# bioinfologics/w2rap-contigger

Hardware: AMD Instinct MI355X
Metric: step2_k60_canonical_kmers_per_s (higher is better)
Workload: dtype u64

## Files before the change

include/w2rap_step2.h:

```cpp
#ifndef W2RAP_STEP2_H_
#define W2RAP_STEP2_H_

#include <stddef.h>
#include <stdint.h>

#ifdef __cplusplus
extern "C" {
#endif

#define W2RAP_STEP2_ABI_VERSION 3

enum {
    W2RAP_OK = 0,
    W2RAP_E_ARG = 1,
    W2RAP_E_NO_DEVICE = 2,
    W2RAP_E_HIP = 3,
    W2RAP_E_STATE = 4,
    W2RAP_E_LIMIT = 5,
    W2RAP_E_GRAPH = 6,
    W2RAP_E_HINT = 7,
    W2RAP_E_IO = 8
};

enum { W2RAP_MEM_HOST = 0, W2RAP_MEM_DEVICE = 1 };
// ... 81 lines not shown
const char* w2rap_step2_last_error(const w2rap_step2_ctx*);
int w2rap_step2_set_reads(w2rap_step2_ctx*, const w2rap_reads* reads);
int w2rap_step2_count_kmers(w2rap_step2_ctx*, uint32_t min_qual, uint32_t min_freq, w2rap_step2_out* stats);
int w2rap_step2_count_kmers_passes(w2rap_step2_ctx*, uint32_t min_qual, uint32_t min_freq, uint32_t n_passes, w2rap_step2_out* stats);
int w2rap_step2_build_graph(w2rap_step2_ctx*, const w2rap_edge_hint* hint);
int w2rap_step2_path_reads(w2rap_step2_ctx*);
int w2rap_step2_fetch(w2rap_step2_ctx*, w2rap_step2_out* out);
void* w2rap_step2_stream(w2rap_step2_ctx*);

int w2rap_step2_trim(w2rap_step2_ctx*);

int w2rap_step2_copy_bench(w2rap_step2_ctx*, uint64_t nbytes, uint32_t reps, double* gb_per_s);
int w2rap_step2_device_copy(w2rap_step2_ctx*, void* dst, const void* src, uint64_t nbytes);
int w2rap_step2_copy_bench_form(void);

int    w2rap_step2_set_profiling(w2rap_step2_ctx*, int on);
size_t w2rap_step2_profile(w2rap_step2_ctx*, char* buf, size_t len, int reset);

int w2rap_step2_counts(w2rap_step2_ctx*, uint64_t out[8]);

int w2rap_step2_get_good_len(w2rap_step2_ctx*, uint16_t* out );
int w2rap_step2_get_table(w2rap_step2_ctx*, uint64_t* hi, uint64_t* lo, uint8_t* count, uint8_t* ctx,
                          int32_t* edge, uint32_t* off );

int      w2rap_step2_quality_windows(w2rap_step2_ctx*, uint32_t min_qual, uint64_t* n_kmers );
uint32_t w2rap_step2_default_buckets(uint64_t total_kmers, uint32_t multiple_of);
uint32_t w2rap_step2_record_bytes(void);
int w2rap_step2_partition(w2rap_step2_ctx*, uint32_t n_buckets, uint32_t n_parts, uint64_t* recs_per_part,
                          uint64_t* kmers_per_part);
int w2rap_step2_partition_range(w2rap_step2_ctx*, uint32_t n_buckets, uint32_t first_bucket, uint32_t end_bucket, uint32_t n_parts,
                                uint64_t* recs_per_part, uint64_t* kmers_per_part);
int w2rap_step2_count_pass(w2rap_step2_ctx*, uint32_t pass, uint32_t n_passes);
int w2rap_step2_partition_buffers(w2rap_step2_ctx*, void** d_records, void** d_bucket_counts, uint64_t* n_records);
int w2rap_step2_count_records(w2rap_step2_ctx*, uint32_t min_freq, uint32_t n_local_buckets, uint32_t n_segments,
                              const void* d_records, const void* d_counts, uint64_t total_kmers, w2rap_step2_out* stats);
int w2rap_step2_count_records_begin(w2rap_step2_ctx*, uint32_t min_freq, uint32_t n_local_buckets, uint32_t n_segments,
                                    const void* d_records, const void* d_counts, uint64_t total_kmers, uint32_t n_slices,
                                    int deferred);
int w2rap_step2_count_records_slices(w2rap_step2_ctx*);
int w2rap_step2_count_records_bounds(w2rap_step2_ctx*, uint32_t k, uint32_t* first_bucket, uint32_t* end_bucket);
int w2rap_step2_count_records_launch(w2rap_step2_ctx*, uint32_t k);
int w2rap_step2_count_records_slice(w2rap_step2_ctx*, uint32_t k, uint64_t* n_solid, uint64_t* n_chunks);
int w2rap_step2_count_records_end(w2rap_step2_ctx*, w2rap_step2_out* stats);
int w2rap_step2_solid_buffers(w2rap_step2_ctx*, void** d_hi, void** d_lo, void** d_cc, uint64_t* n);
int w2rap_step2_set_solid(w2rap_step2_ctx*, const void* d_hi, const void* d_lo, const void* d_cc, uint64_t n,
                          uint64_t M, uint64_t D, const uint64_t* hist101);
// ... 37 lines not shown
```

w2rap_contigger_amd/csrc/ctx.h:

```cpp
#pragma once
#include <hip/hip_runtime.h>
#include <stdint.h>
#include <stdio.h>
#include <stdlib.h>
#include <cstdlib>
#include <string>
#include <utility>
#include <vector>
#include "../../include/w2rap_step2.h"
#include "common.h"

namespace w2 {

struct Ctx;
}
struct w2rap_step2_ctx;
namespace w2 {
struct Ctx {
    int device = 0;
    hipStream_t stream = nullptr;
    hipStream_t stream2 = nullptr;
    unsigned long long* h_pinned = nullptr;
    std::string err;
    int sm_count = 256;
// ... 22 lines not shown
    uint64_t* d_shi = nullptr;
    uint64_t* d_slo = nullptr;
    uint32_t* d_scc = nullptr;
    Slot* d_table = nullptr;
    uint64_t tcap = 0;
    unsigned long long* d_filter32 = nullptr;
    uint64_t f32words = 0;
    uint8_t* d_sctx = nullptr;
    void* d_nbr = nullptr;
    bool wide_ids = false;
    uint64_t* d_chunk_start = nullptr;
    uint32_t* d_chunk_cnt = nullptr;
    uint64_t nchunks = 0;
    KRec* d_srec = nullptr;
    bool use_index = false;
    uint4* d_index = nullptr;
    uint64_t index_cap = 0, index_entries = 0;
    uint4* d_xindex = nullptr; uint64_t xindex_cap = 0, xindex_kmers = 0;
    bool index_prebuilt = false, bits_ready = false, filter_prebuilt = false;
    unsigned cs_ns = 0;
    unsigned cs_planned = 0;
    uint32_t cs_nbl = 0, cs_nseg = 0; const uint32_t* cs_recs = nullptr;
    bool cs_short_first = false;
    hipEvent_t cs_ev[16] = {};
    unsigned long long* cs_cnt = nullptr;
    uint64_t* cs_off = nullptr;
    uint32_t cs_chunk_cap = 0;
    uint8_t* d_unres = nullptr;
    bool fused_prune = false;
    std::vector<std::pair<uint64_t, uint64_t>> unfused_chunks;
    uint32_t* cs_defer = nullptr;
    uint64_t* g_hi = nullptr; uint64_t* g_lo = nullptr; uint32_t* g_cc = nullptr;
    uint64_t* g_cstart = nullptr; uint32_t* g_ccnt = nullptr;
    uint64_t g_cap = 0, g_n = 0, g_ccap = 0, g_nc = 0;
    bool g_open = false;
    hipEvent_t g_copied = nullptr;
    bool quality_done = false, counted = false, graphed = false, pathed_done = false;
    bool table_built = false;

    uint64_t E = 0;
    uint64_t rank_ends = 0;
    uint32_t* d_edge_nk = nullptr;
    uint64_t* d_edge_off = nullptr;
    uint8_t* d_edge_codes = nullptr;
    uint8_t* d_edge_bits = nullptr;
    uint64_t edge_bases = 0;
// ... 208 lines not shown
}
#include <functional>
namespace w2 {
void host_parallel_for(size_t n, const std::function<void(size_t)>& f);

int phase_count(Ctx& c, uint32_t min_qual, uint32_t min_freq);
int count_quality(Ctx& c, uint32_t min_qual);
uint32_t default_buckets(uint64_t total_kmers, uint32_t multiple_of);
int count_partition(Ctx& c, uint32_t nb, uint32_t n_parts, uint32_t pb_lo, uint32_t pb_hi);
int count_buckets(Ctx& c, uint32_t min_freq, uint32_t nbl, uint32_t nseg, const uint32_t* d_recs, const uint32_t* d_counts, uint64_t total_kmers,
                  bool build_table = false);
int count_buckets_launch(Ctx& c, uint32_t min_freq, uint32_t nbl, uint32_t nseg, const uint32_t* d_recs, const uint32_t* d_counts, uint64_t total_kmers,
                         unsigned n_slices, bool deferred);
int count_buckets_launch_slice(Ctx& c, unsigned k);
void count_slice_bounds(const Ctx& c, unsigned k, uint32_t* b_lo, uint32_t* b_hi);
int count_buckets_slice(Ctx& c, unsigned k, uint64_t* n_solid, uint64_t* n_chunks);
int count_buckets_finish(Ctx& c);
int dict_begin(Ctx& c, uint64_t kmer_cap, uint64_t chunk_cap);
int dict_append(Ctx& c, const uint64_t* d_hi, const uint64_t* d_lo, const uint32_t* d_cc, uint64_t n, const uint64_t* d_cstart, const uint32_t* d_ccnt, uint64_t nc,
                uint64_t chunk_bias = 0);
int dict_end(Ctx& c);
void dict_abort(Ctx& c);
int count_table(Ctx& c);
int phase_graph(Ctx& c, const w2rap_edge_hint* hint);
int phase_path(Ctx& c);
int local_dict_slice(Ctx& c, uint64_t n_solid, uint64_t expected_total);
int shard_begin(Ctx& c, unsigned rank, unsigned world, const uint64_t* solid_per_rank, uint32_t n_buckets, uint32_t n_passes, const w2rap_edge_hint* hint);
int shard_next(Ctx& c, w2rap_xchg* x);
int shard_recv(Ctx& c, const uint64_t* recv_count, uint32_t elem_bytes, void** d_recv);
int shard_host_words(Ctx& c, const uint64_t* words);
int shard_info(Ctx& c, uint64_t out[8]);
void shard_free(Ctx& c);
int index_hard_slice(Ctx& c, const uint4* d_all, uint64_t n_all, unsigned rank, unsigned world, uint4** d_hard, uint64_t* n_hard);
int index_hard_apply(Ctx& c, const uint4* d_hard, uint64_t n_hard);
int index_harden(Ctx& c);
int build_index(Ctx& c);
int index_entries_slice(Ctx& c, unsigned rank, unsigned world, uint4** d_list, uint64_t* n_list);
int index_from_entries(Ctx& c, const uint4* d_all, uint64_t n_all, bool harden = true);
uint64_t filter32_words(const Ctx& c);
int filter32_slice(Ctx& c, unsigned rank, unsigned world, unsigned long long** d_slice, uint64_t* n_words);
EdgeIndex edge_index(const Ctx& c);
int index_probe_all(Ctx& c, int32_t* d_edge, uint32_t* d_off);
int run_ranking(Ctx& c, uint64_t N, const uint32_t* nxt0, uint32_t* nxt, uint32_t* rnk, unsigned long long* w, uint8_t* cyc, uint8_t* mid,
                uint32_t* d_flags, const uint64_t* shi, const uint64_t* slo, bool use_chunks);
int decode_pq(Ctx& c, const uint8_t* d_pq, const uint64_t* d_pqoff, uint8_t* d_quals, const uint64_t* d_qoff);

// ... 14 lines not shown
```

w2rap_contigger_amd/csrc/step2_capi.hip:

```cpp
#include <algorithm>
#include <chrono>
#include <cstdlib>
#include <cstring>
#include "ctx.h"

using namespace w2;


namespace {

void set_err(char* err, size_t errlen, const std::string& m) {
    if (err && errlen) { std::snprintf(err, errlen, "%s", m.c_str()); }
}


__global__ void __launch_bounds__(256) k_obj_len(uint64_t NO, const uint32_t* __restrict__ obj_edge, const uint32_t* __restrict__ edge_nk,
                                                  uint32_t* __restrict__ len, uint32_t* __restrict__ nbytes) {
    uint64_t o = (uint64_t)blockIdx.x * blockDim.x + threadIdx.x;
    if (o >= NO) return;
    uint32_t l = edge_nk[obj_edge[o] >> 1] + (K - 1);
    len[o] = l; nbytes[o] = (l + 3) >> 2;
}
__global__ void __launch_bounds__(256) k_pack_objs(uint64_t total_bytes, uint64_t NO, const uint64_t* __restrict__ byte_off,
                                                    const uint32_t* __restrict__ obj_edge, const uint32_t* __restrict__ edge_nk,
// ... 18 lines not shown
    out[i] = (uint8_t)v;
}


}
namespace w2 {
void drop_reads(Ctx& c) {
    (void)quals_wait(c);
    if (c.copy_stream) (void)hipStreamSynchronize(c.copy_stream);
    c.d_qmask = nullptr; c.qmask_min_qual = -1; c.quals_absent = false;
    for (void* p : c.owned_reads) c.park(p);
    c.owned_reads.clear();
    c.d_bases = nullptr; c.d_boff = nullptr; c.d_len = nullptr; c.d_quals = nullptr; c.d_qoff = nullptr; c.n = 0;
}
void drop_results(Ctx& c) {
    if (c.stream) (void)hipStreamSynchronize(c.stream);
    if (c.stream2) (void)hipStreamSynchronize(c.stream2);
    shard_free(c);
    c.free_all();
    c.d_good = nullptr; c.d_bcount = nullptr; c.d_bbase = nullptr; c.d_recs = nullptr; c.d_shi = c.d_slo = nullptr; c.d_scc = nullptr;
    c.d_table = nullptr; c.d_filter32 = nullptr; c.f32words = 0; c.d_sctx = nullptr; c.d_nbr = nullptr; c.d_srec = nullptr; c.d_index = nullptr; c.index_cap = 0; c.d_xindex = nullptr; c.xindex_cap = 0; c.d_unres = nullptr; c.fused_prune = false; c.unfused_chunks.clear();
    c.d_chunk_start = nullptr; c.d_chunk_cnt = nullptr; c.nchunks = 0;
    for (unsigned k = 0; k < c.cs_ns; ++k) (void)hipEventDestroy(c.cs_ev[k]);
    c.cs_ns = 0; c.cs_planned = 0; c.cs_cnt = nullptr; c.cs_off = nullptr; c.cs_defer = nullptr; c.pass = 0; c.npass = 1; c.pass_cnt = nullptr;
    c.g_hi = c.g_lo = nullptr; c.g_cc = nullptr; c.g_cstart = nullptr; c.g_ccnt = nullptr; c.g_open = false; c.g_n = c.g_nc = 0;
    c.d_edge_nk = nullptr; c.d_edge_off = nullptr; c.d_edge_codes = nullptr; c.d_edge_bits = nullptr; c.d_fwdX = c.d_revX = nullptr; c.d_obj_edge = nullptr;
    c.d_otab = nullptr; c.d_left = c.d_right = nullptr; c.d_from_off = c.d_to_off = nullptr; c.d_from_v = c.d_from_e = c.d_to_v = c.d_to_e = nullptr;
    c.d_path_offset = nullptr; c.d_path_off = nullptr; c.d_path_edges = nullptr;
    c.quality_done = c.counted = c.graphed = c.pathed_done = false; c.table_built = false;
    c.M = c.D = c.S = c.E = c.NO = c.NV = 0; c.path_total = 0; c.n_pathed = c.n_multipathed = 0;
}
}
namespace {

template <class T>
int up(Ctx& c, const T** dev, const T* host, uint64_t n, uint64_t pad = 0) {
    T* p = c.alloc<T>(n + pad + 1, false);
    if (!p) return W2RAP_E_HIP;
    c.owned_reads.push_back(p);
    W2_HIP(hipMemsetAsync(p + n, 0, (pad + 1) * sizeof(T), c.stream));
    if (n) W2_TRY(pump_upload(c, p, host, n * sizeof(T)));
    *dev = (const T*)p;
    return 0;
}

}

// ... 552 lines not shown
int w2rap_step2_set_profiling(w2rap_step2_ctx* h, int on) {
    if (!h) return W2RAP_E_ARG;
    h->c.profiling = on != 0;
    return 0;
}

size_t w2rap_step2_profile(w2rap_step2_ctx* h, char* buf, size_t len, int reset) {
    if (!h) return 0;
    std::string s;
    for (auto& x : h->c.prof_sums) s += x.name + " " + std::to_string(x.ms) + " " + std::to_string(x.launches) + "\n";
    if (buf && len) std::snprintf(buf, len, "%s", s.c_str());
    if (reset) h->c.prof_sums.clear();
    return s.size() + 1;
}

int w2rap_step2_get_good_len(w2rap_step2_ctx* h, uint16_t* out) {
    if (!h || !out) return W2RAP_E_ARG;
    Ctx& c = h->c;
    if (!c.counted) { c.err = "get_good_len before count_kmers"; return W2RAP_E_STATE; }
    if (c.n) W2_HIP(hipMemcpy(out, c.d_good, c.n * 2, hipMemcpyDeviceToHost));
    return 0;
}

int w2rap_step2_get_table(w2rap_step2_ctx* h, uint64_t* hi, uint64_t* lo, uint8_t* count, uint8_t* ctx, int32_t* edge, uint32_t* off) {
    if (!h) return W2RAP_E_ARG;
    Ctx& c = h->c;
    if (!c.counted) { c.err = "get_table before count_kmers"; return W2RAP_E_STATE; }
    const uint64_t S = c.S;
    if (!S) return 0;
    if (hi) W2_HIP(hipMemcpy(hi, c.d_shi, S * 8, hipMemcpyDeviceToHost));
    if (lo) W2_HIP(hipMemcpy(lo, c.d_slo, S * 8, hipMemcpyDeviceToHost));
    if (count || (ctx && !c.counted)) {
        std::vector<uint32_t> cc(S);
        W2_HIP(hipMemcpy(cc.data(), c.d_scc, S * 4, hipMemcpyDeviceToHost));
        if (count) for (uint64_t i = 0; i < S; ++i) count[i] = (uint8_t)(cc[i] & 0xFF);
    }
    if (ctx) W2_HIP(hipMemcpy(ctx, c.d_sctx, S, hipMemcpyDeviceToHost));
    if (edge || off) {
        if (!c.graphed) { for (uint64_t i = 0; i < S; ++i) { if (edge) edge[i] = -1; if (off) off[i] = 0; } }
        else if (c.d_srec) {
            std::vector<KRec> sv(S);
            W2_HIP(hipMemcpy(sv.data(), c.d_srec, S * sizeof(KRec), hipMemcpyDeviceToHost));
            for (uint64_t i = 0; i < S; ++i) {
                if (edge) edge[i] = sv[i].kdef.x != NONE32 ? (int32_t)(sv[i].kdef.x & 0x7FFFFFFFu) : -1;
                if (off) off[i] = sv[i].kdef.y;
            }
// ... 122 lines not shown
```

w2rap_contigger_amd/csrc/step2_count.hip:

```cpp
#include <algorithm>
#include <chrono>
#include <cstdlib>
#include <cstring>
#include <type_traits>
#include "ctx.h"

namespace w2 {

constexpr unsigned QSLOTS = 256;
template <bool MASK>
__global__ void __launch_bounds__(256) k_good_len(uint64_t n, const uint8_t* __restrict__ quals, const uint32_t* __restrict__ qmask,
                                                   const uint64_t* __restrict__ qoff, const uint32_t* __restrict__ len,
                                                   uint32_t min_qual, uint16_t* __restrict__ good,
                                                   unsigned long long* __restrict__ total_kmers,
                                                   uint32_t* __restrict__ max_len) {
    constexpr unsigned CH = 4096;
    __shared__ __attribute__((aligned(16))) uint16_t gbits[CH + 16];
    __shared__ unsigned long long s_sum[4];
    __shared__ uint32_t s_max[4];
    const uint64_t r0 = (uint64_t)blockIdx.x * blockDim.x;
    const uint64_t r = r0 + threadIdx.x;
    const uint64_t rend = r0 + blockDim.x < n ? r0 + blockDim.x : n;
    const uint64_t base0 = qoff[r0], endo = qoff[rend];
    const unsigned shift = MASK ? (unsigned)(base0 & 31) : (unsigned)((reinterpret_cast<uintptr_t>(quals) + base0) & 15);
// ... 1022 lines not shown
struct FpKey { uint64_t hi, lo; bool rc; uint32_t f[4]; };
__device__ inline FpKey fp_key(const FpInst& x) {
    auto rev2_32 = [](uint32_t v) { v = __brev(v); return ((v & 0x55555555u) << 1) | ((v >> 1) & 0x55555555u); };
    const uint32_t a0 = rev2_32(x.s[0]), b0 = rev2_32(x.s[1]), a1 = rev2_32(x.s[2]), b1 = rev2_32(x.s[3]);
    FpKey k;
    k.f[0] = a0 >> 4; k.f[1] = __funnelshift_r(b0, a0, 4); k.f[2] = a1 >> 4; k.f[3] = __funnelshift_r(b1, a1, 4);
    const uint64_t khi_f = ((uint64_t)k.f[0] << 32) | k.f[1], klo_f = ((uint64_t)k.f[2] << 32) | k.f[3];
    const uint64_t khi_r = ((uint64_t)(~x.s[3] & 0x0FFFFFFFu) << 32) | (uint32_t)~x.s[2], klo_r = ((uint64_t)(~x.s[1] & 0x0FFFFFFFu) << 32) | (uint32_t)~x.s[0];
    k.rc = khi_r != khi_f ? khi_r < khi_f : klo_r < klo_f;
    k.hi = k.rc ? khi_r : khi_f; k.lo = k.rc ? klo_r : klo_f;
    return k;
}
__device__ inline uint32_t fp_hash(const FpKey& k) {
    const uint32_t fa = (uint32_t)k.hi ^ (uint32_t)(k.lo >> 32), fb = (uint32_t)(k.hi >> 32) ^ (uint32_t)k.lo;
    return (fa + ((fb << 16) | (fb >> 16))) * 0x9E3779B1u;
}
__device__ inline bool fp_same(const uint32_t* tile, unsigned ref, const FpInst& x, const FpKey& k) {
    const FpInst r = fp_fetch(tile, ref >> 6, ref & 63u);
    const uint32_t same = (r.s[0] ^ x.s[0]) | (r.s[1] ^ x.s[1]) | (r.s[2] ^ x.s[2]) | (r.s[3] ^ x.s[3]);
    const uint32_t opp = ((r.s[3] ^ k.f[0]) | 0xF0000000u) & (r.s[2] ^ k.f[1]) & ((r.s[1] ^ k.f[2]) | 0xF0000000u) & (r.s[0] ^ k.f[3]);
    return same == 0u || opp == 0xFFFFFFFFu;
}

template <unsigned THREADS, unsigned MINW, unsigned TILE_, unsigned SC_>
__global__ void __launch_bounds__(THREADS, MINW) k_count_fp(uint32_t nb, uint32_t b_lo, uint32_t b_hi, uint32_t nseg, const uint64_t* __restrict__ roff,
                                                            const uint32_t* __restrict__ recs, uint32_t min_freq, uint32_t* __restrict__ queue,
                                                            uint64_t* __restrict__ shi, uint64_t* __restrict__ slo, uint32_t* __restrict__ scc, uint64_t solid_cap,
                                                            unsigned long long* __restrict__ counters, unsigned long long* __restrict__ ghist,
                                                            uint64_t* __restrict__ chunk_start, uint32_t* __restrict__ chunk_cnt, uint32_t chunk_cap,
                                                            uint32_t* __restrict__ defer , uint32_t defer_cap,
                                                            uint32_t fill_limit , uint32_t solid_limit ,
                                                            uint8_t* __restrict__ sctx, uint8_t* __restrict__ unres, uint32_t* __restrict__ nbr ) {
    constexpr unsigned long long SMASK = (1ull << 40) - 1;
    using C = FpCfg<THREADS, TILE_, SC_>;
    constexpr unsigned CAP = C::CAP, NW = C::NW, TILE = C::TILE, ROUNDS = C::ROUNDS, NPF = C::NPF, SC = C::SC, MAXSEG = C::MAXSEG, PER = C::PER, QCAP = C::QCAP,
                       MAXK = C::MAXK, MAXWIN = C::MAXWIN;
    constexpr uint32_t EMPTY = 0xFFFFFFFFu;
    extern __shared__ __attribute__((aligned(16))) unsigned char smem[];
    uint64_t* segbase = reinterpret_cast<uint64_t*>(smem);
    uint32_t* tab = reinterpret_cast<uint32_t*>(segbase + 3 * MAXSEG);
    uint32_t* cc = tab + CAP;
    uint32_t* tile = cc + CAP;
    uint32_t* bv32 = tile + TILE * FP_TS + 8;
    uint32_t* Bw = bv32 + MAXK / 32 + 2;
    uint32_t* stcc = Bw + MAXWIN + 2;
    uint32_t* stref = stcc + SC;
    uint32_t* qref = stref + SC + (threadIdx.x >> 6) * QCAP;
    uint32_t* segdpre = stref + SC + NW * QCAP;
    uint32_t* wtot = segdpre + 3 * (MAXSEG + 1);
    uint32_t* bq = wtot + 32;
    uint32_t* lhist = bq + 4;
    uint32_t* misc = lhist + 104;
    uint32_t* stk = misc + 16;
    uint16_t* olist = reinterpret_cast<uint16_t*>(stk + 40);
    const unsigned tid = threadIdx.x, lane = tid & 63, wv = tid >> 6;
// ... 55 lines not shown
        const unsigned shl_p = (x.e0 & 3u) ^ (rc ? 3u : 4u), shl_s = ((x.e3 >> 26) & 3u) ^ (rc ? 7u : 0u);
        return (hasp ? 1u << shl_p : 0u) | (hass ? 1u << shl_s : 0u);
    };

    for (unsigned i = tid; i < CAP; i += THREADS) { tab[i] = EMPTY; cc[i] = 0; }
    for (unsigned i = tid; i < MAXK / 32 + 2; i += THREADS) bv32[i] = 0;
    for (unsigned i = tid; i < TILE * FP_TS + 8; i += THREADS) tile[i] = 0;
    for (unsigned i = tid; i < 104; i += THREADS) lhist[i] = 0;
    if (tid < 16) misc[tid] = 0;
    if (tid == 0) {
        const uint32_t t0 = atomicAdd(queue, 3u), nbk = b_hi - b_lo;
        bq[0] = t0 < nbk ? b_lo + t0 : NONE32; bq[1] = t0 + 1 < nbk ? b_lo + t0 + 1 : NONE32; bq[2] = t0 + 2 < nbk ? b_lo + t0 + 2 : NONE32; bq[3] = NONE32;
    }
    __syncthreads();
    if (wv == 0) {
        uint64_t r0; uint32_t cnt;
        seg_load(bq[0], r0, cnt); seg_store(0, r0, cnt);
        seg_load(bq[1], r0, cnt); seg_store(1, r0, cnt);
    }
    __syncthreads();
    uint32_t pf[NPF];
    tile_load(0, pf);
    unsigned long long my_distinct = 0;
    unsigned qn = 0;
    uint32_t tick4 = 0;

    auto drain = [&](unsigned cnt) -> unsigned {
        wave_lds_fence();
        const bool live = lane < cnt;
        const unsigned ref = live ? qref[qn - cnt + lane] : 0u;
        const unsigned rec = ref >> 6, idx = ref & 63u;
        const FpInst x = fp_fetch(tile, rec, idx);
        const FpKey k = fp_key(x);
        const unsigned ctx = ctx_of(x, k.rc, tile[rec * FP_TS], idx);
        const uint32_t h1 = fp_hash(k), tag = (h1 >> 5) & 0xFFFFu;
        unsigned s = (h1 >> (33 - C::LOG_CAP)) << 1;
        bool isnew = false;
        if (live) {
            bool ok = false;
            int budget = (int)CAP;
            for (;;) {
                uint32_t a = ld32(&tab[s]);
                if (a == EMPTY) {
                    a = atomicCAS(&tab[s], EMPTY, (tag << 16) | ref);
                    if (a == EMPTY) { isnew = true; ok = true; break; }
                }
// ... 195 lines not shown
            if (sb) {
                uint32_t base = 0;
                if (lane == (unsigned)__builtin_ctzll(sb)) base = atomicAdd(&misc[FP_CNT], (uint32_t)__builtin_popcountll(sb));
                base = (uint32_t)__builtin_amdgcn_readlane((int)base, (int)__builtin_ctzll(sb));
                if (solid) {
                    const unsigned pos = base + (unsigned)__builtin_popcountll(sb & ((1ull << lane) - 1));
                    stref[pos] = tab[slot] & 0xFFFFu; stcc[pos] = cnt | ((v >> 24) << 8);
                    if (sctx) cc[slot] = 0x80000000u | pos;
                }
            }
            if (live && sctx && !solid) cc[slot] = 0x40000000u;
            if (live && !sctx) { cc[slot] = 0; tab[slot] = EMPTY; }
        }
        __syncthreads();
        {
            const unsigned long long gb = ((unsigned long long)misc[FP_BASELO] | ((unsigned long long)misc[FP_BASEHI] << 32)) & SMASK;
            for (unsigned i0 = 0; i0 < tot; i0 += THREADS) {
                const unsigned i = i0 + tid;
                const bool have = i < tot;
                const uint32_t ref = have ? stref[i] : 0u;
                const FpKey k = fp_key(fp_fetch(tile, ref >> 6, ref & 63u));
                const uint32_t ccv = have ? stcc[i] : 0u;
                if (have && gb + i < solid_cap) { shi[gb + i] = k.hi; slo[gb + i] = k.lo; scc[gb + i] = ccv; }
                if (sctx) {
                    constexpr uint32_t NONE = 0xFFFFFFFFu, PAL = 0xFFFFFFFEu;
                    unsigned c = (ccv >> 8) & 0xFFu, un = 0;
                    uint32_t ns = NONE, np_ = NONE;
                    const Kmer kk{k.hi, k.lo};
                    for (unsigned rest = have ? c : 0u; __any(rest != 0);) {
                        if (rest) {
                            const unsigned t = (unsigned)__builtin_ctz(rest);
                            rest &= rest - 1;
                            Kmer nk = t < 4 ? kmer_succ(kk, t & 3) : kmer_pred(kk, t & 3);
                            const bool r = kmer_canon(nk);
                            FpInst nx; FpKey nkk;
                            const uint64_t lh = rev2_64(nk.hi) >> 4, ll = rev2_64(nk.lo) >> 4;
                            nx.s[0] = (uint32_t)lh; nx.s[1] = (uint32_t)(lh >> 32); nx.s[2] = (uint32_t)ll; nx.s[3] = (uint32_t)(ll >> 32); nx.e0 = 0; nx.e3 = 0;
                            nkk.hi = nk.hi; nkk.lo = nk.lo; nkk.rc = false;
                            nkk.f[0] = (uint32_t)(nk.hi >> 32); nkk.f[1] = (uint32_t)nk.hi; nkk.f[2] = (uint32_t)(nk.lo >> 32); nkk.f[3] = (uint32_t)nk.lo;
                            const uint32_t h1 = fp_hash(nkk), tag = (h1 >> 5) & 0xFFFFu;
                            unsigned s = (h1 >> (33 - C::LOG_CAP)) << 1;
                            int found = -1;
                            for (int budget = (int)CAP; budget > 0; --budget) {
                                const uint32_t a = tab[s];
                                if (a == EMPTY) break;
                                if ((a >> 16) == tag && fp_same(tile, a & 0xFFFFu, nx, nkk)) { found = (int)s; break; }
// ... 7 lines not shown
                                    if (t < 4) ns = id; else np_ = id;
                                } else c &= ~(1u << t);
                            }
                        }
                    }
                    if (have && gb + i < solid_cap) {
                        const unsigned long long gi = gb + i;
                        sctx[gi] = (uint8_t)c; unres[gi] = (uint8_t)un;
                        nbr[2 * gi] = (!(un & 15u) && popc4(c & 15) != 1) ? NONE : ns;
                        nbr[2 * gi + 1] = (!(un >> 4) && popc4(c >> 4) != 1) ? NONE : np_;
                    }
                }
            }
        }
        __syncthreads();
        if (sctx) {
            for (unsigned i = tid; i < tot_occ; i += THREADS) { const unsigned slot = olist[i]; cc[slot] = 0; tab[slot] = EMPTY; }
            if (sp != 0) __syncthreads();
        }
        if (sp == 0) break;
        }
        for (unsigned i = tid; i < 2 * nwin + 2; i += THREADS) bv32[i] = 0;
    }
    __syncthreads();
    for (unsigned i = tid; i < 101; i += THREADS) if (lhist[i]) atomicAdd(&ghist[i], (unsigned long long)lhist[i]);
    for (int o = 32; o > 0; o >>= 1) my_distinct += __shfl_down(my_distinct, o);
    if (lane == 0 && my_distinct) atomicAdd(&counters[1], my_distinct);
}

__global__ void __launch_bounds__(256) k_table_insert(uint64_t i0, uint64_t S, const uint64_t* __restrict__ shi, const uint64_t* __restrict__ slo,
                                                       Slot* __restrict__ table, uint64_t mask) {
    uint64_t i = i0 + (uint64_t)blockIdx.x * blockDim.x + threadIdx.x;
    if (i >= S) return;
    const uint64_t h = kmer_hash(Kmer{shi[i], slo[i]});
    const Slot v = slot_make(h, i);
    uint64_t s = h & mask;
    while (atomicCAS(&table[s], SLOT_EMPTY, v) != SLOT_EMPTY) s = (s + 1) & mask;
}

template <unsigned U> struct PlCfg { static constexpr unsigned CAP = 256 * U, SLOTS = 512 * U, BITS = U == 2 ? 10 : U == 4 ? 11 : 12; };
template <unsigned BITS>
__device__ inline unsigned pl_hash(Kmer k) {
    const uint32_t fa = (uint32_t)k.hi ^ (uint32_t)(k.lo >> 32), fb = (uint32_t)(k.hi >> 32) ^ (uint32_t)k.lo;
    return ((fa + ((fb << 16) | (fb >> 16))) * 0x9E3779B1u) >> (32 - BITS);
}
template <class Id, unsigned U = 2>
__global__ void __launch_bounds__(256) k_prune_local(uint64_t nchunks, const uint64_t* __restrict__ cstart, const uint32_t* __restrict__ ccnt,
                                                      const uint64_t* __restrict__ shi, const uint64_t* __restrict__ slo,
                                                      const uint32_t* __restrict__ scc, uint8_t* __restrict__ sctx,
                                                      Id* __restrict__ nbr, uint8_t* __restrict__ unres) {
    constexpr Id NONE = NodeId<Id>::NONE, PAL = NodeId<Id>::PAL;
    constexpr unsigned PL_CAP = PlCfg<U>::CAP, PL_SLOTS = PlCfg<U>::SLOTS, PL_BITS = PlCfg<U>::BITS;
    __shared__ uint64_t khi[PL_SLOTS], klo[PL_SLOTS];
    __shared__ uint16_t kix[PL_SLOTS];
    const unsigned tid = threadIdx.x;
    auto load_desc = [&](uint64_t ch, uint64_t& st_, uint32_t& cn_) {
        st_ = 0; cn_ = 0;
        if (ch < nchunks) { st_ = cstart[ch]; cn_ = ccnt[ch]; if (cn_ > PL_CAP) cn_ = 0; }
    };
    auto load_keys = [&](uint64_t st_, uint32_t cn_, Kmer (&k_)[U], unsigned (&c_)[U]) {
// ... 394 lines not shown
    uint32_t chunk_cap = c.pass ? c.cs_chunk_cap : 0;
    if (!c.pass) {
        W2_ALLOC(d_cnt, unsigned long long, 160);
        W2_HIP(hipMemsetAsync(d_cnt, 0, 160 * sizeof(unsigned long long), st));
        c.solid_cap = total_kmers / (min_freq ? min_freq : 1) + 1;
        for (void* p : {(void*)c.d_shi, (void*)c.d_slo, (void*)c.d_scc}) if (p) c.release(p);
        W2_ALLOC(c.d_shi, uint64_t, c.solid_cap);
        W2_ALLOC(c.d_slo, uint64_t, c.solid_cap);
        W2_ALLOC(c.d_scc, uint32_t, c.solid_cap);
        if (c.d_chunk_start) { c.release(c.d_chunk_start); c.release(c.d_chunk_cnt); c.d_chunk_start = nullptr; c.d_chunk_cnt = nullptr; }
        c.nchunks = 0;
        if (!getenv("W2RAP_NO_LOCAL_PRUNE")) {
            const uint64_t nb_all = c.npass > 1 ? c.NB : nbl;
            chunk_cap = (uint32_t)std::min<uint64_t>(nb_all * 2 + 4096, 1u << 24);
            W2_ALLOC(c.d_chunk_start, uint64_t, chunk_cap);
            W2_ALLOC(c.d_chunk_cnt, uint32_t, chunk_cap);
            W2_HIP(hipMemsetAsync(c.d_chunk_cnt, 0, (size_t)chunk_cap * 4, st));
        }
    }
    c.cs_cnt = d_cnt; c.cs_off = d_off; c.cs_chunk_cap = chunk_cap;
    W2_ALLOC(c.cs_defer, uint32_t, (uint64_t)nbl + 2);
    c.cs_planned = NS; c.cs_ns = 0; c.cs_nbl = nbl; c.cs_nseg = nseg; c.cs_recs = d_recs;
    c.cs_short_first = deferred && NS >= 3;
    if (!deferred) for (unsigned k = 0; k < NS; ++k) W2_TRY(count_buckets_launch_slice(c, k));
    return 0;
}

void count_slice_bounds(const Ctx& c, unsigned k, uint32_t* b_lo, uint32_t* b_hi) {
    const uint64_t NS = c.cs_planned, nbl = c.cs_nbl;
    auto cut = [&](uint64_t j) -> uint32_t {
        if (!c.cs_short_first) return (uint32_t)(nbl * j / NS);
        return (uint32_t)(j == 0 ? 0 : nbl * (2 * j - 1) / (2 * NS - 1));
    };
    *b_lo = cut(k); *b_hi = cut(k + 1);
}

int count_buckets_launch_slice(Ctx& c, unsigned k) {
    hipStream_t st = c.stream;
    if (!c.cs_planned || k != c.cs_ns || k >= c.cs_planned) { c.err = "count_records_launch: slices are launched once each, in order"; return W2RAP_E_STATE; }
    const unsigned NS = c.cs_planned;
    const uint32_t nbl = c.cs_nbl, nseg = c.cs_nseg;
    unsigned long long* d_cnt = c.cs_cnt;
#ifndef W2RAP_QUEUE_AT
#define W2RAP_QUEUE_AT 144
#endif
    uint32_t* d_queue = reinterpret_cast<uint32_t*>(d_cnt + W2RAP_QUEUE_AT);
    uint32_t b_lo, b_hi;
    count_slice_bounds(c, k, &b_lo, &b_hi);
    auto slice_done = [&]() -> int {
        W2_HIP(hipMemcpyAsync(c.h_pinned + k, d_cnt + 4, 8, hipMemcpyDeviceToHost, st));
        W2_HIP(hipEventCreateWithFlags(&c.cs_ev[k], hipEventDisableTiming));
        W2_HIP(hipEventRecord(c.cs_ev[k], st));
        c.cs_ns = k + 1;
        return 0;
    };
    auto launch = [&](auto kern, unsigned lds, unsigned threads, unsigned blocks_per_cu) -> int {
        W2_HIP(hipFuncSetAttribute(reinterpret_cast<const void*>(kern), hipFuncAttributeMaxDynamicSharedMemorySize, lds));
        unsigned grid = (unsigned)std::min<uint64_t>(b_hi - b_lo, (uint64_t)c.sm_count * blocks_per_cu);
        if (k || c.pass) W2_HIP(hipMemsetAsync(d_queue, 0, 4, st));
        LAUNCH(c, "k_count_buckets", kern, dim3(grid ? grid : 1), dim3(threads), lds, nbl, b_lo, b_hi, nseg, c.cs_off, c.cs_recs, c.min_freq, d_queue,
               c.d_shi, c.d_slo, c.d_scc, c.solid_cap, d_cnt + 4, d_cnt + 8, c.d_chunk_start, c.d_chunk_cnt, c.cs_chunk_cap, (const uint32_t*)nullptr, 0u);
        W2_HIP(hipGetLastError());
        return slice_done();
    };
    auto launch_fp = [&](auto kern, unsigned lds, unsigned threads, unsigned blocks_per_cu, uint32_t fp_limit, uint32_t fp_sc) -> int {
        W2_HIP(hipFuncSetAttribute(reinterpret_cast<const void*>(kern), hipFuncAttributeMaxDynamicSharedMemorySize, lds));
        auto list_kern = k_count_buckets<COUNT_CAP, COUNT_THREADS>;
        W2_HIP(hipFuncSetAttribute(reinterpret_cast<const void*>(list_kern), hipFuncAttributeMaxDynamicSharedMemorySize, (int)K3Cfg<COUNT_CAP, COUNT_THREADS>::LDS));
        const unsigned grid = (unsigned)std::min<uint64_t>(b_hi - b_lo, (uint64_t)c.sm_count * blocks_per_cu);
        if (k || c.pass) W2_HIP(hipMemsetAsync(d_queue, 0, 4, st));
        if (k == 0) W2_HIP(hipMemsetAsync(c.cs_defer, 0, 8, st));
        uint32_t fill_limit = fp_limit, solid_limit = fp_sc;
        if (const char* t = getenv("W2RAP_TEST_FP_LIMIT")) { if (test_hook("W2RAP_TEST_FP_LIMIT")) fill_limit = std::min<uint32_t>(fill_limit, (uint32_t)std::max(1, atoi(t))); }
        if (const char* t = getenv("W2RAP_TEST_FP_SC")) { if (test_hook("W2RAP_TEST_FP_SC")) solid_limit = std::min<uint32_t>(solid_limit, (uint32_t)std::max(1, atoi(t))); }
        LAUNCH(c, "k_count_fp", kern, dim3(grid ? grid : 1), dim3(threads), lds, nbl, b_lo, b_hi, nseg, c.cs_off, c.cs_recs, c.min_freq, d_queue,
               c.d_shi, c.d_slo, c.d_scc, c.solid_cap, d_cnt + 4, d_cnt + 8, c.d_chunk_start, c.d_chunk_cnt, c.cs_chunk_cap, c.cs_defer, nbl, fill_limit, solid_limit,
               c.fused_prune ? c.d_sctx : (uint8_t*)nullptr, c.fused_prune ? c.d_unres : (uint8_t*)nullptr, c.fused_prune ? (uint32_t*)c.d_nbr : (uint32_t*)nullptr);
        W2_HIP(hipGetLastError());
        if (k + 1 == NS && c.fused_prune) W2_HIP(hipMemcpyAsync(c.h_pinned + 20, d_cnt + 4, 8, hipMemcpyDeviceToHost, st));
        if (k + 1 == NS) {
            const unsigned lgrid = (unsigned)std::min<uint64_t>(nbl, (uint64_t)c.sm_count);
            constexpr unsigned list_lds = K3Cfg<COUNT_CAP, COUNT_THREADS>::LDS;
            LAUNCH(c, "k_count_buckets", list_kern, dim3(lgrid ? lgrid : 1), dim3(COUNT_THREADS), list_lds, nbl, 0u, nbl, nseg, c.cs_off,
                   c.cs_recs, c.min_freq, c.cs_defer + 1, c.d_shi, c.d_slo, c.d_scc, c.solid_cap, d_cnt + 4, d_cnt + 8, c.d_chunk_start, c.d_chunk_cnt, c.cs_chunk_cap,
                   (const uint32_t*)c.cs_defer, nbl);
            W2_HIP(hipGetLastError());
        }
        return slice_done();
    };
    const char* v = getenv("W2RAP_K3");
    int cfg = v ? atoi(v) : 22;
    if (cfg >= 20 && nseg > FpCfg<512, 512, 1024>::MAXSEG) cfg = 0;
    if (cfg == 20) W2_TRY(launch_fp(k_count_fp<512, 4, 640, 768>, FpCfg<512, 640, 768>::LDS, 512, 2, FpCfg<512, 640, 768>::LIMIT, 768));
    else if (cfg == 21) W2_TRY(launch_fp(k_count_fp<1024, 8, 576, 512>, FpCfg<1024, 576, 512>::LDS, 1024, 2, FpCfg<1024, 576, 512>::LIMIT, 512));
    else if (cfg == 22) W2_TRY(launch_fp(k_count_fp<512, 4, 512, 1024>, FpCfg<512, 512, 1024>::LDS, 512, 2, FpCfg<512, 512, 1024>::LIMIT, 1024));
    else if (cfg == 23) W2_TRY(launch_fp(k_count_fp<1024, 4, 576, 1024>, FpCfg<1024, 576, 1024>::LDS, 1024, 1, FpCfg<1024, 576, 1024>::LIMIT, 1024));
    else if (cfg == 24) W2_TRY(launch_fp(k_count_fp<512, 4, 576, 1024>, FpCfg<512, 576, 1024>::LDS, 512, 2, FpCfg<512, 576, 1024>::LIMIT, 1024));
    else if (cfg == 1) W2_TRY(launch(k_count_buckets<2048, 512>, K3Cfg<2048, 512>::LDS, 512, 2));
    else if (cfg == 2) W2_TRY(launch(k_count_buckets<4096, 512>, K3Cfg<4096, 512>::LDS, 512, 1));
    else if (cfg == 3) W2_TRY(launch(k_count_buckets<1024, 256>, K3Cfg<1024, 256>::LDS, 256, 4));
    else if (cfg == 5) W2_TRY(launch(k_count_buckets<2048, 1024, false, false, 8>, K3Cfg<2048, 1024, false>::LDS, 1024, 2));
    else if (cfg == 8) W2_TRY(launch(k_count_buckets<4096, 1024, false, false, 1>, K3Cfg<4096, 1024, false>::LDS, 1024, 1));
// ... 38 lines not shown
        fprintf(stderr, "\n");
    }
    if (getenv("W2RAP_TRACE") && h_all[121])
        fprintf(stderr, "[w2rap] k_count_buckets wave-0 clocks per window: loads %.0f, extract+hash %.0f, probe %.0f, atomics %.0f (%.0f windows per block)\n",
                (double)h_all[117] / h_all[121], (double)h_all[118] / h_all[121], (double)h_all[119] / h_all[121], (double)h_all[120] / h_all[121],
                (double)h_all[121] / c.sm_count);
    if (h_all[7]) { c.err = "k_count_buckets: a bucket did not fit the LDS table after 2^16-way splitting"; return W2RAP_E_LIMIT; }
    c.S = h_all[4] & ((1ull << 40) - 1); c.D = h_all[5];
    c.nchunks = c.cs_chunk_cap ? std::min<uint64_t>(h_all[4] >> 40, c.cs_chunk_cap) : 0;
    for (int i = 0; i < 101; ++i) c.hist[i] = h_all[8 + i];
    if (c.S > c.solid_cap) { c.err = "solid k-mer count exceeds its bound"; return W2RAP_E_LIMIT; }
    return 0;
}

static int table_alloc(Ctx& c, uint64_t S, hipStream_t on) {
    uint64_t tcap;
    table_geometry(S, tcap);
    c.tcap = tcap;
    W2_ALLOC(c.d_table, Slot, tcap);
    W2_HIP(hipMemsetAsync(c.d_table, 0xFF, tcap * sizeof(Slot), on));
    return 0;
}

int count_buckets(Ctx& c, uint32_t min_freq, uint32_t nbl, uint32_t nseg, const uint32_t* d_recs, const uint32_t* d_counts,
                  uint64_t total_kmers, bool build_table) {
    hipStream_t st2 = c.stream2;
    const char* nsv = getenv("W2RAP_SLICES");
    unsigned NS = (build_table && !getenv("W2RAP_NO_OVERLAP") && nbl >= 4096 && st2) ? (nsv ? (unsigned)atoi(nsv) : 4) : 1;
    {
        const char* fv = getenv("W2RAP_FUSED_PRUNE"); const char* kv = getenv("W2RAP_K3"); const char* wv = getenv("W2RAP_WIDE_IDS");
        const uint64_t cap = total_kmers / (min_freq ? min_freq : 1) + 1;
        c.fused_prune = build_table && fv && atoi(fv) == 1 && !(kv && atoi(kv) < 20) && !(wv && atoi(wv) != 0) && cap < (1ull << 31) - 1 && c.npass == 1 &&
                        nseg <= 16 && !getenv("W2RAP_NO_LOCAL_PRUNE");
        c.unfused_chunks.clear();
        if (c.fused_prune) {
            for (void* p : {(void*)c.d_sctx, (void*)c.d_nbr, (void*)c.d_unres}) if (p) c.release(p);
            W2_ALLOC(c.d_sctx, uint8_t, cap); W2_ALLOC(c.d_unres, uint8_t, cap);
            uint32_t* nb32 = nullptr; W2_ALLOC(nb32, uint32_t, 2 * cap); c.d_nbr = nb32;
            W2_HIP(hipMemsetAsync(c.d_sctx, 0xFF, cap, c.stream));
            W2_HIP(hipMemsetAsync(c.d_unres, 0xFF, cap, c.stream));
        }
    }
    W2_TRY(count_buckets_launch(c, min_freq, nbl, nseg, d_recs, d_counts, total_kmers, NS, false));
    NS = c.cs_ns;
    uint64_t s_cap = 0;
    if (NS > 1) {
        uint64_t s_prev = 0;
        for (unsigned k = 0; k < NS; ++k) {
            uint64_t s_k = 0;
            W2_TRY(count_buckets_slice(c, k, &s_k, nullptr));
            if (k == 0) {
                s_cap = s_k * NS + s_k / 2 + 1024;
                if (test_hook("W2RAP_TEST_SMALL_SCAP")) s_cap = s_k + 1;
                W2_TRY(table_alloc(c, s_k * NS, st2));
            }
            const uint64_t s_hi = s_k < s_cap ? s_k : s_cap;
            if (s_hi > s_prev) {
                LAUNCH_ON(c, st2, "k_table_insert", k_table_insert, dim3((unsigned)((s_hi - s_prev + 255) / 256)), dim3(256), 0, s_prev, s_hi,
                          c.d_shi, c.d_slo, c.d_table, c.tcap - 1);
                W2_HIP(hipGetLastError());
                s_prev = s_hi;
            }
        }
    }
    W2_TRY(count_buckets_finish(c));
// ... 105 lines not shown
        W2_HIP(hipGetLastError());
        c.ld_done = n_solid;
    }
    return 0;
}
int prune_local_chunks64(Ctx& c, uint8_t* sctx, uint64_t* nbr, uint8_t* unres) {
    hipStream_t st = c.stream;
    W2_HIP(hipMemsetAsync(unres, 0xFF, c.S, st));
    W2_HIP(hipMemsetAsync(sctx, 0xFF, c.S, st));
    if (!c.nchunks || getenv("W2RAP_NO_LOCAL_PRUNE")) return 0;
    const unsigned gl = (unsigned)std::min<uint64_t>(c.nchunks, (uint64_t)c.sm_count * 64);
    PL_LAUNCH(c, uint64_t, gl, c.S, c.nchunks, c.d_chunk_start, c.d_chunk_cnt, c.d_shi, c.d_slo, c.d_scc, sctx, nbr, unres);
    W2_HIP(hipGetLastError());
    return 0;
}
int prune_local_chunks32(Ctx& c, uint8_t* sctx, uint32_t* nbr, uint8_t* unres) {
    hipStream_t st = c.stream;
    W2_HIP(hipMemsetAsync(unres, 0xFF, c.S, st));
    W2_HIP(hipMemsetAsync(sctx, 0xFF, c.S, st));
    if (!c.nchunks || getenv("W2RAP_NO_LOCAL_PRUNE")) return 0;
    const unsigned gl = (unsigned)std::min<uint64_t>(c.nchunks, (uint64_t)c.sm_count * 64);
    PL_LAUNCH(c, uint32_t, gl, c.S, c.nchunks, c.d_chunk_start, c.d_chunk_cnt, c.d_shi, c.d_slo, c.d_scc, sctx, nbr, unres);
    W2_HIP(hipGetLastError());
    return 0;
}

template <class Id>
static int count_table_t(Ctx& c) {
    hipStream_t st = c.stream;
    if (!c.table_built) W2_TRY(table_alloc(c, c.S, st));
    const bool fused = c.fused_prune && sizeof(Id) == 4 && c.d_sctx && c.d_nbr && c.d_unres;
    Id* nbr = nullptr;
    if (fused) nbr = reinterpret_cast<Id*>(c.d_nbr);
    else {
        for (void* p : {(void*)c.d_sctx, (void*)c.d_nbr, (void*)c.d_unres}) if (p) c.release(p);
        c.d_unres = nullptr;
        W2_ALLOC(c.d_sctx, uint8_t, c.S);
        W2_ALLOC(nbr, Id, 2 * c.S);
        c.d_nbr = nbr;
    }
    c.fused_prune = false;
    if (c.S) {
        unsigned g = (unsigned)((c.S + 255) / 256);
        if (!c.table_built) {
            LAUNCH(c, "k_table_insert", k_table_insert, dim3(g), dim3(256), 0, (uint64_t)0, c.S, c.d_shi, c.d_slo, c.d_table, c.tcap - 1);
            W2_HIP(hipGetLastError());
// ... 90 lines not shown
```

Measured before the change: 40.95 billion.

## Fuse hash-table insertion into solid k-mer emission in the counting kernel

Adds an emit-insert path that runs counting in two slices. The first slice is short (1/16 of the buckets) and is used to size the table and is inserted separately on the second stream. The second slice's k_count_fp kernel then inserts each emitted solid k-mer into the lookup table directly with bounded linear probing, which avoids separate insert kernels and the re-read of shi/slo. It falls back to a full rebuild if the probe budget is exhausted or the load factor is too high. It also adds a table_check API for verification. The cost is extra atomics in the counting kernel, the loss of the old four-way slice overlap, and a host sync.

Measured after the change: 39.87 billion, median of 6. -2.6%, worse.

```diff
diff --git a/include/w2rap_step2.h b/include/w2rap_step2.h
--- a/include/w2rap_step2.h
+++ b/include/w2rap_step2.h
@@ -127,6 +127,7 @@
 int w2rap_step2_get_good_len(w2rap_step2_ctx*, uint16_t* out );
 int w2rap_step2_get_table(w2rap_step2_ctx*, uint64_t* hi, uint64_t* lo, uint8_t* count, uint8_t* ctx,
                           int32_t* edge, uint32_t* off );
+int w2rap_step2_table_check(w2rap_step2_ctx*, uint64_t* n_found);
 
 int      w2rap_step2_quality_windows(w2rap_step2_ctx*, uint32_t min_qual, uint64_t* n_kmers );
 uint32_t w2rap_step2_default_buckets(uint64_t total_kmers, uint32_t multiple_of);
diff --git a/w2rap_contigger_amd/csrc/ctx.h b/w2rap_contigger_amd/csrc/ctx.h
--- a/w2rap_contigger_amd/csrc/ctx.h
+++ b/w2rap_contigger_amd/csrc/ctx.h
@@ -68,6 +68,9 @@
     unsigned cs_planned = 0;
     uint32_t cs_nbl = 0, cs_nseg = 0; const uint32_t* cs_recs = nullptr;
     bool cs_short_first = false;
+    unsigned cs_first_div = 0;
+    uint64_t cs_ins_cap = 0;
+    unsigned long long* cs_ins_ctl = nullptr;
     hipEvent_t cs_ev[16] = {};
     unsigned long long* cs_cnt = nullptr;
     uint64_t* cs_off = nullptr;
@@ -322,6 +325,7 @@
 int dict_end(Ctx& c);
 void dict_abort(Ctx& c);
 int count_table(Ctx& c);
+int table_check(Ctx& c, uint64_t* n_found);
 int phase_graph(Ctx& c, const w2rap_edge_hint* hint);
 int phase_path(Ctx& c);
 int local_dict_slice(Ctx& c, uint64_t n_solid, uint64_t expected_total);
diff --git a/w2rap_contigger_amd/csrc/step2_capi.hip b/w2rap_contigger_amd/csrc/step2_capi.hip
--- a/w2rap_contigger_amd/csrc/step2_capi.hip
+++ b/w2rap_contigger_amd/csrc/step2_capi.hip
@@ -64,7 +64,7 @@
     c.d_table = nullptr; c.d_filter32 = nullptr; c.f32words = 0; c.d_sctx = nullptr; c.d_nbr = nullptr; c.d_srec = nullptr; c.d_index = nullptr; c.index_cap = 0; c.d_xindex = nullptr; c.xindex_cap = 0; c.d_unres = nullptr; c.fused_prune = false; c.unfused_chunks.clear();
     c.d_chunk_start = nullptr; c.d_chunk_cnt = nullptr; c.nchunks = 0;
     for (unsigned k = 0; k < c.cs_ns; ++k) (void)hipEventDestroy(c.cs_ev[k]);
-    c.cs_ns = 0; c.cs_planned = 0; c.cs_cnt = nullptr; c.cs_off = nullptr; c.cs_defer = nullptr; c.pass = 0; c.npass = 1; c.pass_cnt = nullptr;
+    c.cs_ns = 0; c.cs_planned = 0; c.cs_cnt = nullptr; c.cs_off = nullptr; c.cs_defer = nullptr; c.cs_first_div = 0; c.cs_ins_cap = 0; c.cs_ins_ctl = nullptr; c.pass = 0; c.npass = 1; c.pass_cnt = nullptr;
     c.g_hi = c.g_lo = nullptr; c.g_cc = nullptr; c.g_cstart = nullptr; c.g_ccnt = nullptr; c.g_open = false; c.g_n = c.g_nc = 0;
     c.d_edge_nk = nullptr; c.d_edge_off = nullptr; c.d_edge_codes = nullptr; c.d_edge_bits = nullptr; c.d_fwdX = c.d_revX = nullptr; c.d_obj_edge = nullptr;
     c.d_otab = nullptr; c.d_left = c.d_right = nullptr; c.d_from_off = c.d_to_off = nullptr; c.d_from_v = c.d_from_e = c.d_to_v = c.d_to_e = nullptr;
@@ -663,6 +663,11 @@
     return 0;
 }
 
+int w2rap_step2_table_check(w2rap_step2_ctx* h, uint64_t* n_found) {
+    if (!h || !n_found) return W2RAP_E_ARG;
+    return table_check(h->c, n_found);
+}
+
 int w2rap_step2_get_table(w2rap_step2_ctx* h, uint64_t* hi, uint64_t* lo, uint8_t* count, uint8_t* ctx, int32_t* edge, uint32_t* off) {
     if (!h) return W2RAP_E_ARG;
     Ctx& c = h->c;
diff --git a/w2rap_contigger_amd/csrc/step2_count.hip b/w2rap_contigger_amd/csrc/step2_count.hip
--- a/w2rap_contigger_amd/csrc/step2_count.hip
+++ b/w2rap_contigger_amd/csrc/step2_count.hip
@@ -1068,6 +1068,9 @@
     return same == 0u || opp == 0xFFFFFFFFu;
 }
 
+struct FpIns { Slot* table; uint64_t mask, cap; unsigned long long* full; };
+constexpr unsigned FP_PROBES = 1024;
+
 template <unsigned THREADS, unsigned MINW, unsigned TILE_, unsigned SC_>
 __global__ void __launch_bounds__(THREADS, MINW) k_count_fp(uint32_t nb, uint32_t b_lo, uint32_t b_hi, uint32_t nseg, const uint64_t* __restrict__ roff,
                                                             const uint32_t* __restrict__ recs, uint32_t min_freq, uint32_t* __restrict__ queue,
@@ -1076,7 +1079,8 @@
                                                             uint64_t* __restrict__ chunk_start, uint32_t* __restrict__ chunk_cnt, uint32_t chunk_cap,
                                                             uint32_t* __restrict__ defer , uint32_t defer_cap,
                                                             uint32_t fill_limit , uint32_t solid_limit ,
-                                                            uint8_t* __restrict__ sctx, uint8_t* __restrict__ unres, uint32_t* __restrict__ nbr ) {
+                                                            uint8_t* __restrict__ sctx, uint8_t* __restrict__ unres, uint32_t* __restrict__ nbr ,
+                                                            const FpIns ins ) {
     constexpr unsigned long long SMASK = (1ull << 40) - 1;
     using C = FpCfg<THREADS, TILE_, SC_>;
     constexpr unsigned CAP = C::CAP, NW = C::NW, TILE = C::TILE, ROUNDS = C::ROUNDS, NPF = C::NPF, SC = C::SC, MAXSEG = C::MAXSEG, PER = C::PER, QCAP = C::QCAP,
@@ -1178,6 +1182,18 @@
     uint32_t pf[NPF];
     tile_load(0, pf);
     unsigned long long my_distinct = 0;
+    Slot ins_v = 0, ins_o = 0;
+    uint64_t ins_s = 0;
+    bool ins_pend = false;
+    auto ins_finish = [&]() {
+        if (!ins_pend) return;
+        ins_pend = false;
+        for (unsigned budget = FP_PROBES; ins_o != SLOT_EMPTY && ins_o != ins_v;) {
+            if (--budget == 0) { atomicOr(ins.full, 1ull); break; }
+            ins_s = (ins_s + 1) & ins.mask;
+            ins_o = atomicCAS(&ins.table[ins_s], SLOT_EMPTY, ins_v);
+        }
+    };
     unsigned qn = 0;
     uint32_t tick4 = 0;
 
@@ -1419,6 +1435,13 @@
                 const FpKey k = fp_key(fp_fetch(tile, ref >> 6, ref & 63u));
                 const uint32_t ccv = have ? stcc[i] : 0u;
                 if (have && gb + i < solid_cap) { shi[gb + i] = k.hi; slo[gb + i] = k.lo; scc[gb + i] = ccv; }
+                if (ins.table && have && gb + i < ins.cap) {
+                    ins_finish();
+                    const uint64_t h = kmer_hash(Kmer{k.hi, k.lo});
+                    ins_v = slot_make(h, gb + i); ins_s = h & ins.mask;
+                    ins_o = atomicCAS(&ins.table[ins_s], SLOT_EMPTY, ins_v);
+                    ins_pend = true;
+                }
                 if (sctx) {
                     constexpr uint32_t NONE = 0xFFFFFFFFu, PAL = 0xFFFFFFFEu;
                     unsigned c = (ccv >> 8) & 0xFFu, un = 0;
@@ -1472,6 +1495,7 @@
         }
         for (unsigned i = tid; i < 2 * nwin + 2; i += THREADS) bv32[i] = 0;
     }
+    if (ins.table) ins_finish();
     __syncthreads();
     for (unsigned i = tid; i < 101; i += THREADS) if (lhist[i]) atomicAdd(&ghist[i], (unsigned long long)lhist[i]);
     for (int o = 32; o > 0; o >>= 1) my_distinct += __shfl_down(my_distinct, o);
@@ -1486,6 +1510,14 @@
     const Slot v = slot_make(h, i);
     uint64_t s = h & mask;
     while (atomicCAS(&table[s], SLOT_EMPTY, v) != SLOT_EMPTY) s = (s + 1) & mask;
+}
+
+__global__ void __launch_bounds__(256) k_table_check(uint64_t S, const uint64_t* __restrict__ shi, const uint64_t* __restrict__ slo,
+                                                      const Slot* __restrict__ table, uint64_t mask, unsigned long long* __restrict__ found) {
+    const uint64_t i = (uint64_t)blockIdx.x * blockDim.x + threadIdx.x;
+    const bool ok = i < S && table_find(table, mask, shi, slo, Kmer{shi[i], slo[i]}) == (int64_t)i;
+    const unsigned long long b = __ballot(ok);
+    if (b && (threadIdx.x & 63) == (unsigned)__builtin_ctzll(b)) atomicAdd(found, (unsigned long long)__builtin_popcountll(b));
 }
 
 template <unsigned U> struct PlCfg { static constexpr unsigned CAP = 256 * U, SLOTS = 512 * U, BITS = U == 2 ? 10 : U == 4 ? 11 : 12; };
@@ -1926,6 +1958,7 @@
     W2_ALLOC(c.cs_defer, uint32_t, (uint64_t)nbl + 2);
     c.cs_planned = NS; c.cs_ns = 0; c.cs_nbl = nbl; c.cs_nseg = nseg; c.cs_recs = d_recs;
     c.cs_short_first = deferred && NS >= 3;
+    c.cs_first_div = 0; c.cs_ins_cap = 0;
     if (!deferred) for (unsigned k = 0; k < NS; ++k) W2_TRY(count_buckets_launch_slice(c, k));
     return 0;
 }
@@ -1933,6 +1966,10 @@
 void count_slice_bounds(const Ctx& c, unsigned k, uint32_t* b_lo, uint32_t* b_hi) {
     const uint64_t NS = c.cs_planned, nbl = c.cs_nbl;
     auto cut = [&](uint64_t j) -> uint32_t {
+        if (c.cs_first_div && NS > 1) {
+            const uint64_t b1 = nbl / c.cs_first_div;
+            return (uint32_t)(j == 0 ? 0 : b1 + (nbl - b1) * (j - 1) / (NS - 1));
+        }
         if (!c.cs_short_first) return (uint32_t)(nbl * j / NS);
         return (uint32_t)(j == 0 ? 0 : nbl * (2 * j - 1) / (2 * NS - 1));
     };
@@ -1979,9 +2016,10 @@
         if (const char* t = getenv("W2RAP_TEST_FP_SC")) { if (test_hook("W2RAP_TEST_FP_SC")) solid_limit = std::min<uint32_t>(solid_limit, (uint32_t)std::max(1, atoi(t))); }
         LAUNCH(c, "k_count_fp", kern, dim3(grid ? grid : 1), dim3(threads), lds, nbl, b_lo, b_hi, nseg, c.cs_off, c.cs_recs, c.min_freq, d_queue,
                c.d_shi, c.d_slo, c.d_scc, c.solid_cap, d_cnt + 4, d_cnt + 8, c.d_chunk_start, c.d_chunk_cnt, c.cs_chunk_cap, c.cs_defer, nbl, fill_limit, solid_limit,
-               c.fused_prune ? c.d_sctx : (uint8_t*)nullptr, c.fused_prune ? c.d_unres : (uint8_t*)nullptr, c.fused_prune ? (uint32_t*)c.d_nbr : (uint32_t*)nullptr);
+               c.fused_prune ? c.d_sctx : (uint8_t*)nullptr, c.fused_prune ? c.d_unres : (uint8_t*)nullptr, c.fused_prune ? (uint32_t*)c.d_nbr : (uint32_t*)nullptr,
+               FpIns{c.cs_ins_cap ? c.d_table : nullptr, c.tcap - 1, c.cs_ins_cap, c.cs_ins_ctl});
         W2_HIP(hipGetLastError());
-        if (k + 1 == NS && c.fused_prune) W2_HIP(hipMemcpyAsync(c.h_pinned + 20, d_cnt + 4, 8, hipMemcpyDeviceToHost, st));
+        if (k + 1 == NS && (c.fused_prune || c.cs_ins_cap)) W2_HIP(hipMemcpyAsync(c.h_pinned + 20, d_cnt + 4, 8, hipMemcpyDeviceToHost, st));
         if (k + 1 == NS) {
             const unsigned lgrid = (unsigned)std::min<uint64_t>(nbl, (uint64_t)c.sm_count);
             constexpr unsigned list_lds = K3Cfg<COUNT_CAP, COUNT_THREADS>::LDS;
@@ -2066,11 +2104,76 @@
     return 0;
 }
 
+static int count_buckets_emit_insert(Ctx& c, uint32_t min_freq, uint32_t nbl, uint32_t nseg, const uint32_t* d_recs, const uint32_t* d_counts,
+                                     uint64_t total_kmers) {
+    hipStream_t st = c.stream, st2 = c.stream2;
+    constexpr unsigned FIRST_DIV = 16;
+    W2_TRY(count_buckets_launch(c, min_freq, nbl, nseg, d_recs, d_counts, total_kmers, 2, true));
+    c.cs_first_div = FIRST_DIV;
+    W2_ALLOC(c.cs_ins_ctl, unsigned long long, 1);
+    W2_HIP(hipMemsetAsync(c.cs_ins_ctl, 0, sizeof(unsigned long long), st));
+    W2_TRY(count_buckets_launch_slice(c, 0));
+    uint64_t s0 = 0;
+    uint32_t b_lo = 0, b_hi = 0;
+    W2_TRY(count_buckets_slice(c, 0, &s0, nullptr));
+    count_slice_bounds(c, 0, &b_lo, &b_hi);
+    const uint64_t est = b_hi ? s0 * nbl / b_hi : s0;
+    W2_TRY(table_alloc(c, est, st));
+    const uint64_t lim = c.tcap * 10 / 13;
+    uint64_t ins_cap = std::min<uint64_t>(est + est / 8 + 1024, lim);
+    bool rebuild = s0 >= lim;
+    if (test_hook("W2RAP_TEST_SMALL_SCAP")) {
+        ins_cap = s0 + 1;
+        rebuild = rebuild || atoi(getenv("W2RAP_TEST_SMALL_SCAP")) == 2;
+    }
+    if (s0 && !rebuild) {
+        hipEvent_t ev;
+        W2_HIP(hipEventCreateWithFlags(&ev, hipEventDisableTiming));
+        W2_HIP(hipEventRecord(ev, st));
+        W2_HIP(hipStreamWaitEvent(st2, ev, 0));
+        (void)hipEventDestroy(ev);
+        LAUNCH_ON(c, st2, "k_table_insert", k_table_insert, dim3((unsigned)((s0 + 255) / 256)), dim3(256), 0, (uint64_t)0, s0,
+                  c.d_shi, c.d_slo, c.d_table, c.tcap - 1);
+        W2_HIP(hipGetLastError());
+    }
+    c.cs_ins_cap = rebuild ? 0 : ins_cap;
+    const int rc = count_buckets_launch_slice(c, 1);
+    c.cs_ins_cap = 0;
+    W2_TRY(rc);
+    W2_TRY(count_buckets_finish(c));
+    unsigned long long full = 0;
+    W2_HIP(hipMemcpyAsync(&full, c.cs_ins_ctl, sizeof(full), hipMemcpyDeviceToHost, st));
+    W2_HIP(hipStreamSynchronize(st));
+    c.release(c.cs_ins_ctl); c.cs_ins_ctl = nullptr;
+    if (c.fused_prune) c.unfused_chunks.emplace_back(std::min<uint64_t>(c.h_pinned[20] >> 40, c.nchunks), c.nchunks);
+    if (rebuild || full || 10 * c.tcap < 13 * c.S) {
+        W2_HIP(hipStreamSynchronize(st2));
+        c.release(c.d_table);
+        c.d_table = nullptr;
+        return 0;
+    }
+    const uint64_t s_fp = std::min<uint64_t>(c.h_pinned[20] & ((1ull << 40) - 1), c.S), r_lo = std::min<uint64_t>(ins_cap, s_fp);
+    if (c.S > r_lo) {
+        LAUNCH_ON(c, st2, "k_table_insert", k_table_insert, dim3((unsigned)((c.S - r_lo + 255) / 256)), dim3(256), 0, r_lo, c.S, c.d_shi, c.d_slo,
+                  c.d_table, c.tcap - 1);
+        W2_HIP(hipGetLastError());
+    }
+    c.table_built = true;
+    return 0;
+}
+
 int count_buckets(Ctx& c, uint32_t min_freq, uint32_t nbl, uint32_t nseg, const uint32_t* d_recs, const uint32_t* d_counts,
                   uint64_t total_kmers, bool build_table) {
     hipStream_t st2 = c.stream2;
     const char* nsv = getenv("W2RAP_SLICES");
     unsigned NS = (build_table && !getenv("W2RAP_NO_OVERLAP") && nbl >= 4096 && st2) ? (nsv ? (unsigned)atoi(nsv) : 4) : 1;
+    bool emit_ins = false;
+    if (NS > 1 && !nsv && c.npass == 1) {
+        const char* ev = getenv("W2RAP_EMIT_INSERT"); const char* kv = getenv("W2RAP_K3");
+        const int cfg = kv ? atoi(kv) : 22;
+        emit_ins = !(ev && atoi(ev) == 0) && cfg >= 20 && cfg <= 24 && nseg <= FpCfg<512, 512, 1024>::MAXSEG;
+        if (emit_ins) NS = 2;
+    }
     {
         const char* fv = getenv("W2RAP_FUSED_PRUNE"); const char* kv = getenv("W2RAP_K3"); const char* wv = getenv("W2RAP_WIDE_IDS");
         const uint64_t cap = total_kmers / (min_freq ? min_freq : 1) + 1;
@@ -2085,6 +2188,7 @@
             W2_HIP(hipMemsetAsync(c.d_unres, 0xFF, cap, c.stream));
         }
     }
+    if (emit_ins) return count_buckets_emit_insert(c, min_freq, nbl, nseg, d_recs, d_counts, total_kmers);
     W2_TRY(count_buckets_launch(c, min_freq, nbl, nseg, d_recs, d_counts, total_kmers, NS, false));
     NS = c.cs_ns;
     uint64_t s_cap = 0;
@@ -2236,6 +2340,23 @@
     const unsigned gl = (unsigned)std::min<uint64_t>(c.nchunks, (uint64_t)c.sm_count * 64);
     PL_LAUNCH(c, uint32_t, gl, c.S, c.nchunks, c.d_chunk_start, c.d_chunk_cnt, c.d_shi, c.d_slo, c.d_scc, sctx, nbr, unres);
     W2_HIP(hipGetLastError());
+    return 0;
+}
+
+int table_check(Ctx& c, uint64_t* n_found) {
+    *n_found = 0;
+    if (!c.counted || !c.d_table) { c.err = "table_check: no lookup table (before count_kmers, or the index replaced it)"; return W2RAP_E_STATE; }
+    if (!c.S) return 0;
+    unsigned long long* d_found = nullptr;
+    W2_ALLOC(d_found, unsigned long long, 1);
+    W2_HIP(hipMemsetAsync(d_found, 0, 8, c.stream));
+    LAUNCH(c, "k_table_check", k_table_check, dim3((unsigned)((c.S + 255) / 256)), dim3(256), 0, c.S, c.d_shi, c.d_slo, c.d_table, c.tcap - 1, d_found);
+    W2_HIP(hipGetLastError());
+    unsigned long long h = 0;
+    W2_HIP(hipMemcpyAsync(&h, d_found, 8, hipMemcpyDeviceToHost, c.stream));
+    W2_HIP(hipStreamSynchronize(c.stream));
+    c.release(d_found);
+    *n_found = h;
     return 0;
 }
 
```
